# bentotten/radiation_ppo

Measured on AMD Instinct MI355X. Metric: env steps/sec (whole node) at 4096 envs; PPO iters/sec at 1/2/4/8 GPUs, higher is better.
Workload: dtype f32 policy / f64+int32 env

## Files before the change

radiation_ppo_amd/csrc/rs_ppo_grad2.hpp:

```cpp
#pragma once
#include "rs_mlp.hpp"

#define RS_T2 33

#ifdef RS_K7_STAMPS
#define RS_K7_NPH 16
__device__ unsigned long long rs_k7_stamp_table[2][RS_K7_NPH];
#define RS_STAMP_ENTRY const unsigned long long st_rt0 = __builtin_amdgcn_s_memrealtime(); const unsigned long long st_t0 = rs_k7_now();
#define RS_STAMP_DECL unsigned long long st_acc[RS_K7_NPH] = {0}; unsigned long long st_last = rs_k7_now(); st_acc[12] = st_last - st_t0;
#define RS_STAMP_EXIT(net) do { RS_STAMP(13); if ((threadIdx.x & 63) == 0) { st_acc[14] = __builtin_amdgcn_s_memrealtime() - st_rt0; \
                           for (int q = 0; q < RS_K7_NPH; ++q) atomicAdd(&rs_k7_stamp_table[net][q], st_acc[q]); } } while (0)
#define RS_STAMP(i) do { __builtin_amdgcn_sched_barrier(0); asm volatile("; RS_STAMP_MARK " #i); const unsigned long long t_ = rs_k7_now(); st_acc[i] += t_ - st_last; st_last = t_; \
                         __builtin_amdgcn_sched_barrier(0); } while (0)
__device__ __forceinline__ unsigned long long rs_k7_now() {
    unsigned long long t;
    asm volatile("s_memtime %0\n\ts_waitcnt lgkmcnt(0)" : "=s"(t) :: "memory");
    return t;
}
#else
#define RS_STAMP_ENTRY
#define RS_STAMP_DECL
#define RS_STAMP_EXIT(net)
#ifdef RS_K7_NO_PHASE_FENCE
#define RS_STAMP(i) do {} while (0)
#else
#define RS_STAMP(i) __builtin_amdgcn_sched_barrier(0)
#endif
#endif
#define RS_XRAW 400
#define RS_XSC 192
#define RS_G2_WAVE_FLOATS ((64 + 32) * RS_T2 + RS_XRAW + RS_XSC + 64)

__host__ __device__ constexpr int rs_grad2_lds_floats(int nout) {
    return ((rs_mlp_lds_floats(nout) + 3) & ~3) + 2 * 2 * 16 * 64 + 2 * 4 * 64 + 8 * RS_G2_WAVE_FLOATS;
}

__device__ __forceinline__ float rs_other_half(float x, int h) {
    const auto r = __builtin_amdgcn_permlane32_swap(__float_as_uint(x), __float_as_uint(x), false, false);
    return __uint_as_float(h ? r[0] : r[1]);
}

__device__ __forceinline__ void rs_stage32(float* T, const f32x16& v, int c, int h) {
#pragma unroll
    for (int r = 0; r < 16; ++r) T[rs_kappa(r, h) * RS_T2 + c] = v[r];
}

template <int NOUT>
__device__ __forceinline__ void rs_ppo_grad2_body(const RsMlpParams prm, const rs_ppo_batch B, float* partial,
                                                  double* stat_partial, const int* stop,
                                                  const rs_update_state* ust, int* snap,
                                                  const int bid, const int nblocks) {
    extern __shared__ __align__(16) float smem_f[];
    if (snap && bid == 0 && threadIdx.x == 0) { snap[0] = ust->adam_step; snap[1] = ust->stopped; }
    if (stop && *stop) return;
    RS_STAMP_ENTRY
    RsMlpLds<NOUT> W;
    W.carve(smem_f);
    float* w2tf = smem_f + ((rs_mlp_lds_floats(NOUT) + 3) & ~3);
    float* w3tf = w2tf + 2 * 2 * 16 * 64;
    const int wid = __builtin_amdgcn_readfirstlane(threadIdx.x >> 6);
    const int lane = threadIdx.x & 63, h = lane >> 5, c = lane & 31;
    const int l15 = lane & 15, l4 = lane >> 4;
    float* Qt = w3tf + 2 * 4 * 64 + wid * RS_G2_WAVE_FLOATS;
    float* Pt = Qt + 64 * RS_T2;
    float* xraw = Pt + 32 * RS_T2;
    float* xsc = xraw + RS_XRAW;
    float* dbl = xsc + RS_XSC;
    float* w1b = W.w1f;
    for (int i = threadIdx.x; i < 2 * 6 * 64; i += blockDim.x) {
        const int l = i & 63, s = (i >> 6) % 6, it = i / (6 * 64);
        const int row = 32 * it + (l & 31), k = 2 * s + (l >> 5);
        w1b[i] = RS_TANH_PRESCALE * ((k < RS_IN) ? prm.w1[row * RS_IN + k] : prm.b1[row]);
    }
    for (int i = threadIdx.x; i < 2 * 2 * 16 * 64; i += blockDim.x) {
        const int ri = i & 3, l = (i >> 2) & 63, r4 = (i >> 8) & 3, kt = (i >> 10) & 1, it = i >> 11;
        const int r = 4 * r4 + ri;
        w2tf[i] = prm.w2[(32 * kt + rs_kappa(r, l >> 5)) * RS_HID + 32 * it + (l & 31)];
        W.w2f[i] = RS_TANH_PRESCALE * prm.w2[(32 * it + (l & 31)) * RS_HID + 32 * kt + rs_kappa(r, l >> 5)];
    }
    for (int i = threadIdx.x; i < 2 * 4 * 64; i += blockDim.x) {
        int l = i & 63, sq = (i >> 6) & 3, it = i >> 8;
        int o = 2 * sq + (l >> 5);
        w3tf[i] = (o < NOUT) ? prm.w3[o * RS_HID + 32 * it + (l & 31)] : 0.0f;
    }
    for (int i = threadIdx.x; i < 2 * NOUT * 32; i += blockDim.x) {
        const int q = i & 31, o = (i >> 5) % NOUT, hh = i / (32 * NOUT);
        W.w3h[i] = prm.w3[o * RS_HID + 32 * (q >> 4) + rs_kappa(q & 15, hh)];
    }
    for (int i = threadIdx.x; i < 64; i += blockDim.x) W.b2[i] = RS_TANH_PRESCALE * prm.b2[i];
    for (int i = threadIdx.x; i < NOUT; i += blockDim.x) W.b3[i] = prm.b3[i];
    dbl[lane] = 0.0f;
    __syncthreads();

    const int M = B.M;
    const int groups = (M + 31) / 32;
    const int wave_g = bid * 8 + wid, n_waves = nblocks * 8;

    f32x16 acc2[2][2];
    f32x4 acc1[4], acc3[4];
#pragma unroll
    for (int a = 0; a < 2; ++a)
#pragma unroll
        for (int r = 0; r < 16; ++r) { acc2[a][0][r] = 0.f; acc2[a][1][r] = 0.f; }
#pragma unroll
    for (int a = 0; a < 4; ++a)
#pragma unroll
        for (int r = 0; r < 4; ++r) { acc1[a][r] = 0.f; acc3[a][r] = 0.f; }
    f32x4 accs;
#pragma unroll
    for (int r = 0; r < 4; ++r) accs[r] = 0.f;

    const int trips = (groups + n_waves - 1) / n_waves;
    const long x_last = (long)M * RS_IN - 1;
    auto dma_rows = [&](int g) {
        const char* gx = reinterpret_cast<const char*>(B.x + (long)g * (32 * RS_IN));
        const int lim = (int)(x_last - (long)g * (32 * RS_IN));
#pragma unroll
        for (int i = 0; i < 6; ++i) {
            const int o = min(i * 64 + lane, lim);
            __builtin_amdgcn_global_load_lds((const __attribute__((address_space(1))) void*)(gx + 4u * (unsigned)o),
                                             (__attribute__((address_space(3))) void*)(xraw + i * 64), 4, 0, 0);
        }
    };
    auto dma_scal = [&](int g) {
        const int m0 = g * 32;
        const int ms = min(m0 + c, M - 1);
        {
            const int mi = min(m0 + (lane >> 1), M - 1);
            const int* src = reinterpret_cast<const int*>(B.act) + 2 * (size_t)mi + (lane & 1);
            __builtin_amdgcn_global_load_lds((const __attribute__((address_space(1))) void*)src,
                                             (__attribute__((address_space(3))) void*)(xsc), 4, 0, 0);
        }
        {
            const float* src = (h ? B.logp_old : B.adv) + ms;
            __builtin_amdgcn_global_load_lds((const __attribute__((address_space(1))) void*)src,
                                             (__attribute__((address_space(3))) void*)(xsc + 64), 4, 0, 0);
        }
        {
            const float* src = (h ? B.ret : B.w) + ms;
            __builtin_amdgcn_global_load_lds((const __attribute__((address_space(1))) void*)src,
                                             (__attribute__((address_space(3))) void*)(xsc + 128), 4, 0, 0);
        }
    };
    {
        const int g0 = wave_g < groups ? wave_g : groups - 1;
        dma_rows(g0);
        dma_scal(g0);
    }
    RS_STAMP_DECL
    for (int trip = 0; trip < trips; ++trip) {
        RS_STAMP(15);
        const int gi_raw = wave_g + trip * n_waves;
        const int gi = gi_raw < groups ? gi_raw : groups - 1;
        const int m = gi * 32 + c;
        const bool valid = gi_raw < groups && m < M;
        asm volatile("s_waitcnt vmcnt(0)" ::: "memory");
#if defined(RS_K7_ALIGN) && RS_K7_ALIGN >= 1
        __builtin_amdgcn_s_barrier();
#endif
        const float wi = valid ? xsc[128 + c] : 0.0f;
        const int s_act = reinterpret_cast<const int*>(xsc)[2 * c];
        const float s_adv = xsc[64 + c], s_lpo = xsc[96 + c], s_ret = xsc[160 + c];
        float xv[6];
#pragma unroll
        for (int s6 = 0; s6 < 6; ++s6) xv[s6] = xraw[c * RS_IN + 2 * s6 + h];
        if (h) xv[5] = 1.0f;
        RS_STAMP(0);
        f32x16 H1[2], H2[2];
#pragma unroll
        for (int it = 0; it < 2; ++it)
#pragma unroll
            for (int r = 0; r < 16; ++r) H1[it][r] = 0.0f;
        {
            float a0 = w1b[(0 * 6 + 0) * 64 + lane], a1 = w1b[(1 * 6 + 0) * 64 + lane];
#pragma unroll
            for (int s = 0; s < 6; ++s) {
                const float b = xv[s];
                float n0 = 0.f, n1 = 0.f;
                if (s + 1 < 6) { n0 = w1b[(0 * 6 + s + 1) * 64 + lane]; n1 = w1b[(1 * 6 + s + 1) * 64 + lane]; }
                H1[0] = __builtin_amdgcn_mfma_f32_32x32x2f32(a0, b, H1[0], 0, 0, 0);
                H1[1] = __builtin_amdgcn_mfma_f32_32x32x2f32(a1, b, H1[1], 0, 0, 0);
                a0 = n0; a1 = n1;
            }
        }
        RS_STAMP(1);
#pragma unroll
        for (int it = 0; it < 2; ++it)
#pragma unroll
            for (int r = 0; r < 16; ++r) H1[it][r] = rs_tanh_scaled(H1[it][r]);
#pragma unroll
        for (int it = 0; it < 2; ++it)
#pragma unroll
            for (int q = 0; q < 4; ++q) {
                const float4 b = *reinterpret_cast<const float4*>(W.b2 + 32 * it + 8 * q + 4 * h);
                H2[it][4 * q + 0] = b.x; H2[it][4 * q + 1] = b.y; H2[it][4 * q + 2] = b.z; H2[it][4 * q + 3] = b.w;
            }
        RS_STAMP(2);
        {
            const float4* wq = reinterpret_cast<const float4*>(W.w2f) + lane;
            float4 a0 = wq[0], a1 = wq[(1 * 2 + 0) * 4 * 64];
#pragma unroll
            for (int g4 = 0; g4 < 8; ++g4) {
                const int kt = g4 >> 2, r0 = 4 * (g4 & 3);
                float4 n0 = a0, n1 = a1;
                if (g4 + 1 < 8) {
                    n0 = wq[((0 * 2 + ((g4 + 1) >> 2)) * 4 + ((g4 + 1) & 3)) * 64];
                    n1 = wq[((1 * 2 + ((g4 + 1) >> 2)) * 4 + ((g4 + 1) & 3)) * 64];
                }
                H2[0] = __builtin_amdgcn_mfma_f32_32x32x2f32(a0.x, H1[kt][r0 + 0], H2[0], 0, 0, 0);
                H2[1] = __builtin_amdgcn_mfma_f32_32x32x2f32(a1.x, H1[kt][r0 + 0], H2[1], 0, 0, 0);
                H2[0] = __builtin_amdgcn_mfma_f32_32x32x2f32(a0.y, H1[kt][r0 + 1], H2[0], 0, 0, 0);
                H2[1] = __builtin_amdgcn_mfma_f32_32x32x2f32(a1.y, H1[kt][r0 + 1], H2[1], 0, 0, 0);
                H2[0] = __builtin_amdgcn_mfma_f32_32x32x2f32(a0.z, H1[kt][r0 + 2], H2[0], 0, 0, 0);
                H2[1] = __builtin_amdgcn_mfma_f32_32x32x2f32(a1.z, H1[kt][r0 + 2], H2[1], 0, 0, 0);
                H2[0] = __builtin_amdgcn_mfma_f32_32x32x2f32(a0.w, H1[kt][r0 + 3], H2[0], 0, 0, 0);
                H2[1] = __builtin_amdgcn_mfma_f32_32x32x2f32(a1.w, H1[kt][r0 + 3], H2[1], 0, 0, 0);
                a0 = n0; a1 = n1;
            }
        }
        rs_stage32(Qt, H1[0], c, h);
        rs_stage32(Qt + 32 * RS_T2, H1[1], c, h);
        RS_STAMP(3);
#if defined(RS_K7_ALIGN) && RS_K7_ALIGN >= 2
        __builtin_amdgcn_s_barrier();
#endif
#pragma unroll
        for (int it = 0; it < 2; ++it)
#pragma unroll
            for (int r = 0; r < 16; ++r) H2[it][r] = rs_tanh_scaled(H2[it][r]);
        RS_STAMP(4);
        float out[NOUT];
        {
            float pacc[NOUT];
#pragma unroll
            for (int o = 0; o < NOUT; ++o) pacc[o] = 0.0f;
            const float4* wrow = reinterpret_cast<const float4*>(W.w3h + h * NOUT * 32);
            float4 wb[NOUT];
#pragma unroll
            for (int o = 0; o < NOUT; ++o) wb[o] = wrow[o * 8];
#pragma unroll
            for (int b = 0; b < 8; ++b) {
                const int kt = b >> 2, r4 = b & 3;
                float4 wn[NOUT];
#pragma unroll
                for (int o = 0; o < NOUT; ++o) wn[o] = (b + 1 < 8) ? wrow[o * 8 + b + 1] : wb[o];
#pragma unroll
                for (int o = 0; o < NOUT; ++o) {
                    pacc[o] = fmaf(wb[o].x, H2[kt][4 * r4 + 0], pacc[o]);
                    pacc[o] = fmaf(wb[o].y, H2[kt][4 * r4 + 1], pacc[o]);
                    pacc[o] = fmaf(wb[o].z, H2[kt][4 * r4 + 2], pacc[o]);
                    pacc[o] = fmaf(wb[o].w, H2[kt][4 * r4 + 3], pacc[o]);
                }
                if (b + 1 < 8) {
                    __builtin_amdgcn_sched_group_barrier(0x100, NOUT, 0);
                    __builtin_amdgcn_sched_group_barrier(0x002, 4 * NOUT, 0);
                }
#pragma unroll
                for (int o = 0; o < NOUT; ++o) wb[o] = wn[o];
            }
#pragma unroll
            for (int o = 0; o < NOUT; ++o) {
                const float q = rs_other_half(pacc[o], h);
                out[o] = (h ? (q + pacc[o]) : (pacc[o] + q)) + W.b3[o];
            }
        }
        RS_STAMP(5);
        float dz[NOUT], sq[4];
        if (NOUT == 8) {
            const int a = s_act;
            const float adv = s_adv, lpo = s_lpo;
            float mx = out[0];
#pragma unroll
            for (int j = 1; j < NOUT; ++j) mx = fmaxf(mx, out[j]);
            float se = 0.f;
#pragma unroll
            for (int j = 0; j < NOUT; ++j) se += __expf(out[j] - mx);
            const float lse = __logf(se);
            float lp[NOUT], pj[NOUT], ent = 0.f, logp = 0.f;
#pragma unroll
            for (int j = 0; j < NOUT; ++j) {
                lp[j] = (out[j] - mx) - lse;
                pj[j] = __expf(lp[j]);
                ent -= pj[j] * lp[j];
                logp = (a == j) ? lp[j] : logp;
            }
            const float ratio = __expf(logp - lpo);
            const float lo = 1.0f - B.clip_ratio, hi = 1.0f + B.clip_ratio;
            const float clipped = fminf(fmaxf(ratio, lo), hi);
            const float s1 = ratio * adv, s2 = clipped * adv;
            const float surr = fminf(s1, s2);
            const bool inside = ratio >= lo && ratio <= hi;
            const float dr = (inside || s1 < s2) ? adv : 0.0f;
            const float g_lp = -wi * dr * ratio;
#pragma unroll
            for (int j = 0; j < NOUT; ++j) dz[j] = g_lp * (((a == j) ? 1.0f : 0.0f) - pj[j]);
            sq[0] = wi * (lpo - logp);
            sq[1] = wi * ent;
            sq[2] = wi * ((ratio > hi || ratio < lo) ? 1.0f : 0.0f);
            sq[3] = wi * surr;
        } else {
            const float diff = out[0] - s_ret;
            dz[0] = 2.0f * B.vf_coef * wi * diff;
            sq[0] = wi * diff * diff; sq[1] = 0.f; sq[2] = 0.f; sq[3] = 0.f;
        }
        RS_STAMP(6);

        float* Dz = xraw;
        if (h == 0) {
#pragma unroll
            for (int o = 0; o < NOUT; ++o) Dz[o * RS_T2 + c] = dz[o];
        } else {
#pragma unroll
            for (int q = 0; q < 4; ++q) Dz[(8 + q) * RS_T2 + c] = sq[q];
        }
#pragma unroll
        for (int hf = 0; hf < 2; ++hf) {
            rs_wave_sync();
            rs_stage32(Pt, H2[hf], c, h);
            rs_wave_sync();
            const bool a_row = l15 < NOUT || (l15 >= 8 && l15 < 12);
            float a_c = a_row ? Dz[l15 * RS_T2 + l4] : 0.0f;
            float b_c[2];
#pragma unroll
            for (int u = 0; u < 2; ++u) b_c[u] = Pt[(16 * u + l15) * RS_T2 + l4];
#pragma unroll
            for (int s = 0; s < 8; ++s) {
                float a_n = 0.f, b_n[2] = {0.f, 0.f};
                if (s + 1 < 8) {
                    a_n = a_row ? Dz[l15 * RS_T2 + 4 * (s + 1) + l4] : 0.0f;
#pragma unroll
                    for (int u = 0; u < 2; ++u) b_n[u] = Pt[(16 * u + l15) * RS_T2 + 4 * (s + 1) + l4];
                }
                const float a_dz = (l15 < NOUT) ? a_c : 0.0f;
#pragma unroll
                for (int u = 0; u < 2; ++u) acc3[2 * hf + u] = __builtin_amdgcn_mfma_f32_16x16x4f32(a_dz, b_c[u], acc3[2 * hf + u], 0, 0, 0);
                if (hf == 0) accs = __builtin_amdgcn_mfma_f32_16x16x4f32(a_c, 1.0f, accs, 0, 0, 0);
                a_c = a_n;
#pragma unroll
                for (int u = 0; u < 2; ++u) b_c[u] = b_n[u];
            }
        }
        RS_STAMP(7);
        if (NOUT == 8) {
#pragma unroll
            for (int it = 0; it < 2; ++it) {
                f32x16 t;
#pragma unroll
                for (int r = 0; r < 16; ++r) t[r] = 0.f;
#pragma unroll
                for (int s = 0; s < 4; ++s) {
                    const float b = h ? dz[(2 * s + 1) % NOUT] : dz[(2 * s) % NOUT];
                    t = __builtin_amdgcn_mfma_f32_32x32x2f32(w3tf[(it * 4 + s) * 64 + lane], b, t, 0, 0, 0);
                }
#pragma unroll
                for (int r = 0; r < 16; ++r) { const float hv = H2[it][r]; H2[it][r] = fmaf(-(t[r] * hv), hv, t[r]); }
            }
        } else {
#pragma unroll
            for (int kt = 0; kt < 2; ++kt)
#pragma unroll
                for (int r = 0; r < 16; ++r) {
                    const float hv = H2[kt][r];
                    const float d = W.w3h[h * 32 + kt * 16 + r] * dz[0];
                    H2[kt][r] = fmaf(-(d * hv), hv, d);
                }
        }
        {
            const int gn_raw = wave_g + (trip + 1) * n_waves;
            const int gn = gn_raw < groups ? gn_raw : groups - 1;
            asm volatile("s_waitcnt lgkmcnt(0)" ::: "memory");
            dma_rows(gn);
            dma_scal(gn);
        }
        RS_STAMP(8);
#if defined(RS_K7_ALIGN) && RS_K7_ALIGN >= 3
        __builtin_amdgcn_s_barrier();
#endif
        rs_wave_sync();
        rs_stage32(Pt, H2[0], c, h);
        f32x16 D1[2];
#pragma unroll
        for (int it = 0; it < 2; ++it)
#pragma unroll
            for (int r = 0; r < 16; ++r) D1[it][r] = 0.f;
        {
            const float4* wq = reinterpret_cast<const float4*>(w2tf) + lane;
            float4 a0 = wq[0], a1 = wq[(1 * 2 + 0) * 4 * 64];
#pragma unroll
            for (int g4 = 0; g4 < 8; ++g4) {
                const int kt = g4 >> 2, r0 = 4 * (g4 & 3);
                float4 n0 = a0, n1 = a1;
                if (g4 + 1 < 8) {
                    n0 = wq[((0 * 2 + ((g4 + 1) >> 2)) * 4 + ((g4 + 1) & 3)) * 64];
                    n1 = wq[((1 * 2 + ((g4 + 1) >> 2)) * 4 + ((g4 + 1) & 3)) * 64];
                }
                D1[0] = __builtin_amdgcn_mfma_f32_32x32x2f32(a0.x, H2[kt][r0 + 0], D1[0], 0, 0, 0);
                D1[1] = __builtin_amdgcn_mfma_f32_32x32x2f32(a1.x, H2[kt][r0 + 0], D1[1], 0, 0, 0);
                D1[0] = __builtin_amdgcn_mfma_f32_32x32x2f32(a0.y, H2[kt][r0 + 1], D1[0], 0, 0, 0);
                D1[1] = __builtin_amdgcn_mfma_f32_32x32x2f32(a1.y, H2[kt][r0 + 1], D1[1], 0, 0, 0);
                D1[0] = __builtin_amdgcn_mfma_f32_32x32x2f32(a0.z, H2[kt][r0 + 2], D1[0], 0, 0, 0);
                D1[1] = __builtin_amdgcn_mfma_f32_32x32x2f32(a1.z, H2[kt][r0 + 2], D1[1], 0, 0, 0);
                D1[0] = __builtin_amdgcn_mfma_f32_32x32x2f32(a0.w, H2[kt][r0 + 3], D1[0], 0, 0, 0);
                D1[1] = __builtin_amdgcn_mfma_f32_32x32x2f32(a1.w, H2[kt][r0 + 3], D1[1], 0, 0, 0);
                a0 = n0; a1 = n1;
            }
        }
        float xb[8];
        {
            int gi_late = gi;
            asm volatile("" : "+v"(gi_late));
#pragma unroll
            for (int s8 = 0; s8 < 8; ++s8) {
                int n = gi_late * 32 + 4 * s8 + l4;
                n = n < M ? n : M - 1;
                xb[s8] = (l15 < RS_IN) ? B.x[(size_t)n * RS_IN + l15] : ((l15 == RS_IN) ? 1.0f : 0.0f);
            }
        }
#pragma unroll
        for (int it = 0; it < 2; ++it)
#pragma unroll
            for (int r = 0; r < 16; ++r) {
                const float hv = Qt[(32 * it + rs_kappa(r, h)) * RS_T2 + c];
                const float d = D1[it][r];
                D1[it][r] = fmaf(-(d * hv), hv, d);
            }
        rs_wave_sync();
        RS_STAMP(9);
#pragma unroll
        for (int it = 0; it < 2; ++it) {
            if (it == 1) {
                rs_wave_sync();
                rs_stage32(Pt, H2[1], c, h);
                rs_wave_sync();
            }
            float a_c = Pt[c * RS_T2 + h], b0_c = Qt[c * RS_T2 + h], b1_c = Qt[(32 + c) * RS_T2 + h];
#pragma unroll
            for (int s = 0; s < 16; ++s) {
                float a_n = 0.f, b0_n = 0.f, b1_n = 0.f;
                if (s + 1 < 16) {
                    a_n = Pt[c * RS_T2 + 2 * (s + 1) + h];
                    b0_n = Qt[c * RS_T2 + 2 * (s + 1) + h];
                    b1_n = Qt[(32 + c) * RS_T2 + 2 * (s + 1) + h];
                }
                acc2[it][0] = __builtin_amdgcn_mfma_f32_32x32x2f32(a_c, b0_c, acc2[it][0], 0, 0, 0);
                acc2[it][1] = __builtin_amdgcn_mfma_f32_32x32x2f32(a_c, b1_c, acc2[it][1], 0, 0, 0);
                a_c = a_n; b0_c = b0_n; b1_c = b1_n;
            }
            float rs = 0.0f;
#pragma unroll
            for (int n = 0; n < 16; ++n) rs += Pt[c * RS_T2 + 16 * h + n];
            rs += rs_other_half(rs, h);
            if (h == 0) dbl[32 * it + c] += rs;
        }
        RS_STAMP(10);
#pragma unroll
        for (int it = 0; it < 2; ++it) {
            rs_wave_sync();
            rs_stage32(Pt, D1[it], c, h);
            rs_wave_sync();
            float a0_c = Pt[l15 * RS_T2 + l4], a1_c = Pt[(16 + l15) * RS_T2 + l4];
#pragma unroll
            for (int s = 0; s < 8; ++s) {
                float a0_n = 0.f, a1_n = 0.f;
                if (s + 1 < 8) {
                    a0_n = Pt[l15 * RS_T2 + 4 * (s + 1) + l4];
                    a1_n = Pt[(16 + l15) * RS_T2 + 4 * (s + 1) + l4];
                }
                acc1[2 * it + 0] = __builtin_amdgcn_mfma_f32_16x16x4f32(a0_c, xb[s], acc1[2 * it + 0], 0, 0, 0);
                acc1[2 * it + 1] = __builtin_amdgcn_mfma_f32_16x16x4f32(a1_c, xb[s], acc1[2 * it + 1], 0, 0, 0);
                a0_c = a0_n; a1_c = a1_n;
            }
        }
        rs_wave_sync();
        RS_STAMP(11);
    }
    constexpr int RS_REST = rs_net_params(NOUT) - 64 * 64;
    static_assert(8 * 64 * 64 <= rs_grad2_lds_floats(NOUT) && 8 * ((RS_REST + 1) & ~1) + 2 * 8 * 5 <= rs_grad2_lds_floats(NOUT),
                  "the epilogue's slabs must fit K7's LDS");
    int tid_e = threadIdx.x;
    asm volatile("" : "+v"(tid_e));
    const int lane_e = tid_e & 63, h_e = lane_e >> 5, c_e = lane_e & 31, l15_e = lane_e & 15, l4_e = lane_e >> 4;
    asm volatile("s_waitcnt vmcnt(0)" ::: "memory");
    const float db2v = dbl[lane_e];
    __syncthreads();
    float* outp = partial + (size_t)bid * rs_net_params(NOUT);
    {
        float* g_w2 = smem_f + wid * (64 * 64);
#pragma unroll
        for (int it = 0; it < 2; ++it)
#pragma unroll
            for (int r = 0; r < 16; ++r) {
                const int row = 32 * it + rs_kappa(r, h_e);
                g_w2[row * 64 + c_e] = acc2[it][0][r];
                g_w2[row * 64 + 32 + c_e] = acc2[it][1][r];
            }
    }
    __syncthreads();
    for (int i = tid_e; i < 64 * 64; i += blockDim.x) {
        float v = 0.0f + smem_f[i];
#pragma unroll
        for (int wv = 1; wv < 8; ++wv) v += smem_f[wv * (64 * 64) + i];
        outp[64 * RS_IN + 64 + i] = v;
    }
    float db3r[NOUT];
#pragma unroll
    for (int o = 0; o < NOUT; ++o) db3r[o] = __shfl(accs[o & 3], 16 * (o >> 2));
    double sv[5];
    {
        const float t0 = __shfl(accs[0], 32), t1 = __shfl(accs[1], 32), t2 = __shfl(accs[2], 32), t3 = __shfl(accs[3], 32);
        if (NOUT == 8) { sv[0] = (double)t0; sv[1] = (double)t1; sv[2] = (double)t2; sv[3] = 0.0; sv[4] = (double)t3; }
        else { sv[0] = 0.0; sv[1] = 0.0; sv[2] = 0.0; sv[3] = (double)t0; sv[4] = 0.0; }
    }
    constexpr int RS_RSTR = (RS_REST + 1) & ~1;
    double* sred = reinterpret_cast<double*>(smem_f + 8 * RS_RSTR);
    __syncthreads();
    {
        float* g_w1 = smem_f + wid * RS_RSTR, *g_b1 = g_w1 + 64 * RS_IN, *g_b2 = g_b1 + 64, *g_w3 = g_b2 + 64, *g_b3 = g_w3 + NOUT * 64;
        g_b2[lane_e] = db2v;
#pragma unroll
        for (int u = 0; u < 4; ++u)
#pragma unroll
            for (int q = 0; q < 4; ++q) {
                const int row = 16 * u + 4 * l4_e + q;
                if (l15_e < RS_IN) g_w1[row * RS_IN + l15_e] = acc1[u][q];
                if (l15_e == RS_IN) g_b1[row] = acc1[u][q];
                const int o = 4 * l4_e + q;
                if (o < NOUT) g_w3[o * 64 + 16 * u + l15_e] = acc3[u][q];
            }
        if (lane_e == 0) {
#pragma unroll
            for (int o = 0; o < NOUT; ++o) g_b3[o] = db3r[o];
#pragma unroll
            for (int q = 0; q < 5; ++q) sred[wid * 5 + q] = sv[q];
        }
    }
    __syncthreads();
    for (int i = tid_e; i < RS_REST; i += blockDim.x) {
        float v = 0.0f + smem_f[i];
#pragma unroll
        for (int wv = 1; wv < 8; ++wv) v += smem_f[wv * RS_RSTR + i];
        outp[i < 64 * RS_IN + 64 ? i : i + 64 * 64] = v;
    }
    if (tid_e < 5) {
        double v = 0.0 + sred[tid_e];
#pragma unroll
        for (int wv = 1; wv < 8; ++wv) v += sred[wv * 5 + tid_e];
        stat_partial[(size_t)bid * 5 + tid_e] = v;
    }
    RS_STAMP_EXIT(NOUT == 8 ? 0 : 1);
}

template <int NOUT>
__global__ void __launch_bounds__(512, 2) rs_ppo_grad2_kernel(RsMlpParams prm, rs_ppo_batch B, float* __restrict__ partial,
                                                              double* __restrict__ stat_partial, const int* __restrict__ stop,
                                                              const rs_update_state* __restrict__ ust, int* __restrict__ snap) {
    rs_ppo_grad2_body<NOUT>(prm, B, partial, stat_partial, stop, ust, snap, blockIdx.x, gridDim.x);
}

__global__ void __launch_bounds__(512, 2) rs_ppo_grad2_pair_kernel(RsMlpParams pa, RsMlpParams pc, rs_ppo_batch B, float* __restrict__ partial_a,
                                                                   float* __restrict__ partial_c, double* __restrict__ stat_a,
                                                                   double* __restrict__ stat_c, const int* __restrict__ stop,
                                                                   const rs_update_state* __restrict__ ust, int* __restrict__ snap) {
    const int G = gridDim.x >> 1;
    if ((int)blockIdx.x < G) rs_ppo_grad2_body<8>(pa, B, partial_a, stat_a, stop, nullptr, nullptr, blockIdx.x, G);
    else rs_ppo_grad2_body<1>(pc, B, partial_c, stat_c, stop, ust, snap, blockIdx.x - G, G);
}
```

Before: 40.18 million.

## Specialize critic (NOUT=1) gradient path with register weights and 4x4 MFMA outer products

```diff
diff --git a/radiation_ppo_amd/csrc/rs_ppo_grad2.hpp b/radiation_ppo_amd/csrc/rs_ppo_grad2.hpp
--- a/radiation_ppo_amd/csrc/rs_ppo_grad2.hpp
+++ b/radiation_ppo_amd/csrc/rs_ppo_grad2.hpp
@@ -125,13 +125,13 @@
     auto dma_scal = [&](int g) {
         const int m0 = g * 32;
         const int ms = min(m0 + c, M - 1);
-        {
+        if constexpr (NOUT == 8) {
             const int mi = min(m0 + (lane >> 1), M - 1);
             const int* src = reinterpret_cast<const int*>(B.act) + 2 * (size_t)mi + (lane & 1);
             __builtin_amdgcn_global_load_lds((const __attribute__((address_space(1))) void*)src,
                                              (__attribute__((address_space(3))) void*)(xsc), 4, 0, 0);
         }
-        {
+        if constexpr (NOUT == 8) {
             const float* src = (h ? B.logp_old : B.adv) + ms;
             __builtin_amdgcn_global_load_lds((const __attribute__((address_space(1))) void*)src,
                                              (__attribute__((address_space(3))) void*)(xsc + 64), 4, 0, 0);
@@ -146,6 +146,15 @@
         const int g0 = wave_g < groups ? wave_g : groups - 1;
         dma_rows(g0);
         dma_scal(g0);
+    }
+    float w3v[NOUT == 1 ? 32 : 1], db2r[2] = {0.0f, 0.0f};
+    if constexpr (NOUT == 1) {
+        const float4* wrow = reinterpret_cast<const float4*>(W.w3h + h * 32);
+#pragma unroll
+        for (int b = 0; b < 8; ++b) {
+            const float4 t = wrow[b];
+            w3v[4 * b + 0] = t.x; w3v[4 * b + 1] = t.y; w3v[4 * b + 2] = t.z; w3v[4 * b + 3] = t.w;
+        }
     }
     RS_STAMP_DECL
     for (int trip = 0; trip < trips; ++trip) {
@@ -230,7 +239,13 @@
             for (int r = 0; r < 16; ++r) H2[it][r] = rs_tanh_scaled(H2[it][r]);
         RS_STAMP(4);
         float out[NOUT];
-        {
+        if constexpr (NOUT == 1) {
+            float pacc = 0.0f;
+#pragma unroll
+            for (int q = 0; q < 32; ++q) pacc = fmaf(w3v[q], H2[q >> 4][q & 15], pacc);
+            const float q = rs_other_half(pacc, h);
+            out[0] = (h ? (q + pacc) : (pacc + q)) + W.b3[0];
+        } else {
             float pacc[NOUT];
 #pragma unroll
             for (int o = 0; o < NOUT; ++o) pacc[o] = 0.0f;
@@ -306,6 +321,36 @@
         RS_STAMP(6);
 
         float* Dz = xraw;
+        if constexpr (NOUT == 1) {
+            constexpr int T4 = 36;
+            float* zrow = xraw + 96;
+            float* ones = xraw + 160;
+            zrow[32 * h + c] = h ? sq[0] : dz[0];
+            ones[c] = 1.0f;
+            float4 av[8];
+#pragma unroll
+            for (int hf = 0; hf < 2; ++hf) {
+                rs_wave_sync();
+#pragma unroll
+                for (int r = 0; r < 16; ++r) Pt[rs_kappa(r, h) * T4 + c] = H2[hf][r];
+                rs_wave_sync();
+                if (hf == 0) {
+#pragma unroll
+                    for (int q = 0; q < 8; ++q) av[q] = *reinterpret_cast<const float4*>(zrow + 32 * (lane & 1) + 4 * q);
+                }
+                const float* brow = (hf == 0 && h) ? ones : Pt + c * T4;
+                float4 bv[8];
+#pragma unroll
+                for (int q = 0; q < 8; ++q) bv[q] = *reinterpret_cast<const float4*>(brow + 4 * q);
+#pragma unroll
+                for (int q = 0; q < 8; ++q) {
+                    acc3[hf] = __builtin_amdgcn_mfma_f32_4x4x1f32(av[q].x, bv[q].x, acc3[hf], 0, 0, 0);
+                    acc3[hf] = __builtin_amdgcn_mfma_f32_4x4x1f32(av[q].y, bv[q].y, acc3[hf], 0, 0, 0);
+                    acc3[hf] = __builtin_amdgcn_mfma_f32_4x4x1f32(av[q].z, bv[q].z, acc3[hf], 0, 0, 0);
+                    acc3[hf] = __builtin_amdgcn_mfma_f32_4x4x1f32(av[q].w, bv[q].w, acc3[hf], 0, 0, 0);
+                }
+            }
+        } else {
         if (h == 0) {
 #pragma unroll
             for (int o = 0; o < NOUT; ++o) Dz[o * RS_T2 + c] = dz[o];
@@ -340,6 +385,7 @@
                 for (int u = 0; u < 2; ++u) b_c[u] = b_n[u];
             }
         }
+        }
         RS_STAMP(7);
         if (NOUT == 8) {
 #pragma unroll
@@ -361,7 +407,7 @@
 #pragma unroll
                 for (int r = 0; r < 16; ++r) {
                     const float hv = H2[kt][r];
-                    const float d = W.w3h[h * 32 + kt * 16 + r] * dz[0];
+                    const float d = w3v[kt * 16 + r] * dz[0];
                     H2[kt][r] = fmaf(-(d * hv), hv, d);
                 }
         }
@@ -450,7 +496,8 @@
 #pragma unroll
             for (int n = 0; n < 16; ++n) rs += Pt[c * RS_T2 + 16 * h + n];
             rs += rs_other_half(rs, h);
-            if (h == 0) dbl[32 * it + c] += rs;
+            if constexpr (NOUT == 1) db2r[it] += rs;
+            else if (h == 0) dbl[32 * it + c] += rs;
         }
         RS_STAMP(10);
 #pragma unroll
@@ -481,7 +528,7 @@
     asm volatile("" : "+v"(tid_e));
     const int lane_e = tid_e & 63, h_e = lane_e >> 5, c_e = lane_e & 31, l15_e = lane_e & 15, l4_e = lane_e >> 4;
     asm volatile("s_waitcnt vmcnt(0)" ::: "memory");
-    const float db2v = dbl[lane_e];
+    const float db2v = NOUT == 1 ? (h_e ? db2r[1] : db2r[0]) : dbl[lane_e];
     __syncthreads();
     float* outp = partial + (size_t)bid * rs_net_params(NOUT);
     {
@@ -503,13 +550,15 @@
         outp[64 * RS_IN + 64 + i] = v;
     }
     float db3r[NOUT];
-#pragma unroll
-    for (int o = 0; o < NOUT; ++o) db3r[o] = __shfl(accs[o & 3], 16 * (o >> 2));
     double sv[5];
-    {
+    if constexpr (NOUT == 1) {
+        db3r[0] = __shfl(acc3[0][0], 32);
+        sv[0] = 0.0; sv[1] = 0.0; sv[2] = 0.0; sv[3] = (double)__shfl(acc3[0][1], 32); sv[4] = 0.0;
+    } else {
+#pragma unroll
+        for (int o = 0; o < NOUT; ++o) db3r[o] = __shfl(accs[o & 3], 16 * (o >> 2));
         const float t0 = __shfl(accs[0], 32), t1 = __shfl(accs[1], 32), t2 = __shfl(accs[2], 32), t3 = __shfl(accs[3], 32);
-        if (NOUT == 8) { sv[0] = (double)t0; sv[1] = (double)t1; sv[2] = (double)t2; sv[3] = 0.0; sv[4] = (double)t3; }
-        else { sv[0] = 0.0; sv[1] = 0.0; sv[2] = 0.0; sv[3] = (double)t0; sv[4] = 0.0; }
+        sv[0] = (double)t0; sv[1] = (double)t1; sv[2] = (double)t2; sv[3] = 0.0; sv[4] = (double)t3;
     }
     constexpr int RS_RSTR = (RS_REST + 1) & ~1;
     double* sred = reinterpret_cast<double*>(smem_f + 8 * RS_RSTR);
@@ -525,8 +574,9 @@
                 if (l15_e < RS_IN) g_w1[row * RS_IN + l15_e] = acc1[u][q];
                 if (l15_e == RS_IN) g_b1[row] = acc1[u][q];
                 const int o = 4 * l4_e + q;
-                if (o < NOUT) g_w3[o * 64 + 16 * u + l15_e] = acc3[u][q];
-            }
+                if (NOUT == 8 && o < NOUT) g_w3[o * 64 + 16 * u + l15_e] = acc3[u][q];
+            }
+        if (NOUT == 1 && lane_e < 32) { g_w3[lane_e] = acc3[0][0]; g_w3[32 + lane_e] = acc3[1][0]; }
         if (lane_e == 0) {
 #pragma unroll
             for (int o = 0; o < NOUT; ++o) g_b3[o] = db3r[o];
```

After: 41.13 million, median of 6. +2.4%, better.
